# tqch/ddpm-torch

Hardware: AMD Instinct MI355X
Metric: training imgs/s/GPU + 1000-step DDPM samples/s, CIFAR-10 UNet @1/2/4/8 MI355X (higher is better)
Workload: dtype bf16

## Files before the change

### ddpm-torch_amd/csrc/conv3x3.hip

```cpp
#include "common.h"
#include <string.h>
#include <stdlib.h>

namespace {

typedef float f32x4v __attribute__((ext_vector_type(4)));
typedef unsigned u32x2 __attribute__((ext_vector_type(2)));

struct CsArgs {
    const bf16_t* x; long long x_ld; unsigned x_extent;
    const bf16_t* w; unsigned w_extent;
    bf16_t* out; long long out_ld;
    const float* bias; const float* rowbias; long long rowbias_ld; unsigned rowbias_extent;
    const bf16_t* res; long long res_ld;
    int accumulate;
    int B, H, W, C, N, K;
    int ups;
    int tiles_y, tiles_x, tiles_n, total_tiles, xcd;
    FastDiv d_tiles_n, d_tpi, d_tiles_x;
};

template <int PATCH> struct Geo;
template <> struct Geo<16> {
    static constexpr int HWD = 18, HP = 324, LP = 4;
    static constexpr int NI = 6;
    static constexpr int RING = 4;
    static constexpr int WM = 4, NIB = 2, NJ = 2;
    static constexpr int HALO_BYTES = 5 * 512 * 16 + 1024;
};
template <> struct Geo<8> {
    static constexpr int HWD = 10, HP = 100, LP = 3;
    static constexpr int NI = 2;
    static constexpr int RING = 6;
    static constexpr int WM = 2, NIB = 1, NJ = 1;
    static constexpr int HALO_BYTES = 2 * 512 * 16;
};
constexpr int WT_BYTES = 128 * 128;
template <int PATCH> struct Lds {
    static constexpr int DUMP_AT = 2 * Geo<PATCH>::HALO_BYTES + Geo<PATCH>::RING * WT_BYTES;
    static constexpr int ROWS_AT = DUMP_AT + 1024;
    static constexpr int BYTES = ROWS_AT + 4096;
    static_assert(BYTES <= 160 * 1024, "LDS");
};

struct TilePos { int img, py0, px0, tn; };

#ifdef C3_TRACE
__device__ unsigned long long* g_c3_trace = nullptr;
#define C3_TR(id) asm volatile("s_memtime %0" : "=s"(tr_now[id]))
#ifndef C3_TRACE_FIRST
#define C3_TRACE_FIRST 5
#endif
#else
#define C3_TR(id)
#endif
#ifdef C3_TIMING
__device__ unsigned long long* g_c3_timing = nullptr;
#define C3_STAMP(slot) do { if (g_c3_timing && threadIdx.x == 0) g_c3_timing[blockIdx.x * 8 + (slot)] = (slot) == 0 || (slot) == 7 ? wall_clock64() : clock64(); } while (0)
#else
#define C3_STAMP(slot)
#endif

template <int PATCH>
__global__ __launch_bounds__(512, 2)
void conv3x3_stream_kernel(CsArgs a) {
    typedef Geo<PATCH> G_;
    constexpr int HWD = G_::HWD, HP = G_::HP, LP = G_::LP, NI = G_::NI, RING = G_::RING, WM = G_::WM, NIB = G_::NIB, NJ = G_::NJ;
    constexpr int HALO_BYTES = G_::HALO_BYTES, DUMP_AT = Lds<PATCH>::DUMP_AT, ROWS_AT = Lds<PATCH>::ROWS_AT;
    C3_STAMP(0); C3_STAMP(1);
    extern __shared__ __attribute__((aligned(16))) char smem[];
    char* halo = smem;
    char* wring = smem + 2 * HALO_BYTES;
    const int tid = threadIdx.x, lane = tid & 63;
    const int wave = __builtin_amdgcn_readfirstlane(tid >> 6);
    const int wn = wave / WM, wm = wave % WM;

    const __amdgpu_buffer_rsrc_t rx = buffer_rsrc(a.x, a.x_extent), rw = buffer_rsrc(a.w, a.w_extent);
    const __amdgpu_buffer_rsrc_t rbias = buffer_rsrc(a.bias ? (const void*)a.bias : (const void*)a.w, a.bias ? (unsigned)(a.N * 4) : 0u);
    const __amdgpu_buffer_rsrc_t rrow = buffer_rsrc(a.rowbias ? (const void*)a.rowbias : (const void*)a.w, a.rowbias ? a.rowbias_extent : 0u);

    const bool extra = a.res || a.accumulate;
    const int G = gridDim.x;
    const int my_tiles = a.total_tiles > (int)blockIdx.x ? (a.total_tiles - 1 - (int)blockIdx.x) / G + 1 : 0;
    if (my_tiles == 0) return;
    auto tile_pos = [&](int k) {
        const int lid = xcd_logical_id(blockIdx.x + k * G, a.total_tiles, a.xcd);
        const int tmi = (int)fdiv((unsigned)lid, a.d_tiles_n);
        const int tpi = a.tiles_y * a.tiles_x;
        const int img = (int)fdiv((unsigned)tmi, a.d_tpi), pt = tmi - img * tpi;
        const int ty = (int)fdiv((unsigned)pt, a.d_tiles_x);
        TilePos t; t.img = img; t.py0 = ty * PATCH; t.px0 = (pt - ty * a.tiles_x) * PATCH; t.tn = lid - tmi * a.tiles_n;
        return t;
    };
    auto halo_plan = [&](const TilePos& t, unsigned (&ho)[NI]) {
        int tid_ = tid;
        asm volatile("" : "+v"(tid_));
#pragma unroll
        for (int i = 0; i < NI; ++i) {
            const int v = tid_ + 512 * i, hp = v >> 3;
            const int hy = hp / HWD, hx = hp - hy * HWD;
            const int iy = t.py0 + hy - 1, ix = t.px0 + hx - 1;
            const bool ok = hp < HP && (unsigned)iy < (unsigned)a.H && (unsigned)ix < (unsigned)a.W;
            const int lc = (v & 7) ^ (PATCH == 16 ? (hx >> 1) & 7 : ((hx >> 1) ^ ((hy & 1) << 2)) & 7);
            const int sy = iy >> a.ups, sx = ix >> a.ups;
            ho[i] = ok ? ((unsigned)((t.img * (a.H >> a.ups) + sy) * (a.W >> a.ups) + sx) * (unsigned)a.x_ld + (unsigned)(lc * 8)) * 2u : BUF_OOB;
        }
    };
    auto halo_part_off = [&](const TilePos& t, int i) {
        int tid_ = tid;
        asm volatile("" : "+v"(tid_));
        const int v = tid_ + 512 * i, hp = v >> 3;
        const int hy = hp / HWD, hx = hp - hy * HWD;
        const int iy = t.py0 + hy - 1, ix = t.px0 + hx - 1;
        const bool ok = hp < HP && (unsigned)iy < (unsigned)a.H && (unsigned)ix < (unsigned)a.W;
        const int lc = (v & 7) ^ (PATCH == 16 ? (hx >> 1) & 7 : ((hx >> 1) ^ ((hy & 1) << 2)) & 7);
        const int sy = iy >> a.ups, sx = ix >> a.ups;
        return ok ? ((unsigned)((t.img * (a.H >> a.ups) + sy) * (a.W >> a.ups) + sx) * (unsigned)a.x_ld + (unsigned)(lc * 8)) * 2u : BUF_OOB;
    };
    auto issue_halo_part = [&](unsigned ho, int i, int cc, char* dst) {
        const unsigned o = ho == BUF_OOB ? BUF_OOB : ho + (unsigned)(cc * 128);
        char* d = (PATCH == 8 || i < 5) ? dst + (wave * 64 + 512 * i) * 16 : (wave == 0 ? dst + 5 * 512 * 16 : smem + DUMP_AT);
        LDS_DMA16(rx, d, o, 0);
    };
    unsigned wrow[2];
#pragma unroll
    for (int i = 0; i < 2; ++i) {
        const int v = tid + 512 * i, row = v >> 3, lc = (v & 7) ^ ((row >> 1) & 7);
        wrow[i] = (unsigned)(((long long)row * a.K + lc * 8) * 2);
    }
    const unsigned w_tile_bytes = (unsigned)((long long)128 * a.K * 2);
    const int nchunks = a.C >> 6;
    const int steps_per_tile = nchunks * 9, total = my_tiles * steps_per_tile;

    auto issue_w = [&](int tn, int cc, int tap, int slot) {
        char* dst = wring + slot * WT_BYTES;
        const unsigned base = (unsigned)tn * w_tile_bytes + (unsigned)((tap * a.C + cc * 64) * 2);
#pragma unroll
        for (int i = 0; i < 2; ++i)
            LDS_DMA16(rw, dst + (wave * 64 + 512 * i) * 16, base + wrow[i], 0);
    };
    auto issue_w_half = [&](int tn, int cc, int tap, int slot, int i) {
        char* dst = wring + slot * WT_BYTES;
        const unsigned base = (unsigned)tn * w_tile_bytes + (unsigned)((tap * a.C + cc * 64) * 2);
        LDS_DMA16(rw, dst + (wave * 64 + 512 * i) * 16, base + wrow[i], 0);
    };
    auto issue_rows = [&](const TilePos& t, int parity) {
        char* slot = smem + ROWS_AT + parity * 2048;
        if (wave == 0 && a.bias)
            LDS_DMA16(rbias, slot, lane < 32 ? (unsigned)((t.tn * 128 + lane * 4) * 4) : BUF_OOB, 0);
        if (wave == 1 && a.rowbias)
            LDS_DMA16(rrow, slot + 1024, lane < 32 ? (unsigned)(((long long)t.img * a.rowbias_ld + t.tn * 128 + lane * 4) * 4) : BUF_OOB, 0);
    };

    int hp0[NJ], pxl[NJ], pyl[NJ];
#pragma unroll
    for (int j = 0; j < NJ; ++j) {
        const int p = wm * (32 * NJ) + j * 32 + (lane & 31);
        hp0[j] = (p >> LP) * HWD + (p & (PATCH - 1));
        pxl[j] = p & (PATCH - 1); pyl[j] = (p >> LP) & 1;
    }
    f32x16 acc[NIB][NJ];
#pragma unroll
    for (int i = 0; i < NIB; ++i)
#pragma unroll
        for (int j = 0; j < NJ; ++j) acc[i][j] = (f32x16)(0.f);

    TilePos cur = tile_pos(0);
    unsigned hoff[NI];
    halo_plan(cur, hoff);
#pragma unroll
    for (int i = 0; i < NI; ++i) issue_halo_part(hoff[i], i, 0, halo);
    issue_rows(cur, 0);
#pragma unroll
    for (int t = 0; t < RING - 1; ++t) issue_w(cur.tn, 0, t, t);
    wait_vm<2 * (RING - 2)>();
    __builtin_amdgcn_s_barrier();

    C3_STAMP(2);
    const int sw = (lane >> 5) ^ ((lane >> 1) & 7);
    const int hi = lane >> 5;
    const unsigned lds0 = lds_addr(smem);
    unsigned wv[NIB], hv[NJ];
#pragma unroll
    for (int i = 0; i < NIB; ++i) wv[i] = lds0 + 2 * HALO_BYTES + (unsigned)((wn * (32 * NIB) + i * 32 + (lane & 31)) * 128 + (sw << 4));
#pragma unroll
    for (int j = 0; j < NJ; ++j) hv[j] = lds0 + (unsigned)(hp0[j] * 128);
    u32x4 fw[2][NIB], fx[2][NJ];
    bool pend = false;
#ifdef C3_TRACE
    int trace_step = 0;
    unsigned long long tr_now[16], tr_keep[4][16];
#pragma unroll
    for (int q = 0; q < 4; ++q)
#pragma unroll
        for (int i = 0; i < 16; ++i) tr_keep[q][i] = 0;
#endif
    int slot = 0, hb = 0;
    constexpr int ST = NIB * (32 * NJ / 16);
    bool st8 = false;
    for (int k = 0; k < my_tiles; ++k) {
        const bool more_tiles = k + 1 < my_tiles;
        TilePos nxt = cur;
        if (more_tiles) nxt = tile_pos(k + 1);
        for (int cc = 0; cc < nchunks; ++cc) {
            const char* hcur = halo + hb * HALO_BYTES;
            char* hnxt = halo + (hb ^ 1) * HALO_BYTES;
            const bool same_tile = cc + 1 < nchunks;
            const bool prefetch = same_tile || more_tiles;
            const bool last_chunk = !same_tile;
            const int ncc = same_tile ? cc + 1 : 0;
            const int ntn = same_tile ? cur.tn : nxt.tn;
            u32x2 rv[NJ][NIB][4];
            bool pre = false;
#pragma unroll
            for (int tap = 0; tap < 9; ++tap) {
                const int r = tap / 3, s = tap - 3 * r;
                const int shift = r * HWD + s;
                const unsigned woff = (unsigned)(slot * WT_BYTES);
                const unsigned hoffs = (unsigned)(hb * HALO_BYTES + shift * 128);
                unsigned hk[NJ], wk[NIB];
#pragma unroll
                for (int j = 0; j < NJ; ++j) {
                    int px = pxl[j];
                    asm volatile("" : "+v"(px));
                    const int key = PATCH == 16 ? ((px + s) >> 1) & 7 : (((px + s) >> 1) ^ (((pyl[j] + r) & 1) << 2)) & 7;
                    hk[j] = hv[j] + hoffs + (unsigned)((hi ^ key) << 4);
                }
#pragma unroll
                for (int i = 0; i < NIB; ++i) { wk[i] = wv[i]; asm volatile("" : "+v"(wk[i])); }
                auto sub_step = [&](bool mf, const u32x4 (&cw)[NIB], const u32x4 (&cx)[NJ], int kc, u32x4 (&nw)[NIB], u32x4 (&nx)[NJ]) {
                    auto rd_w = [&](int i) {
                        if (kc < 0) return;
                        const unsigned ad = (wk[i] ^ (unsigned)(kc << 5)) + woff;
                        asm volatile("ds_read_b128 %0, %1" : "=v"(nw[i]) : "v"(ad) : "memory");
                        __builtin_amdgcn_sched_barrier(0);
                    };
                    auto rd_x = [&](int j) {
                        if (kc < 0) return;
                        const unsigned ad = hk[j] ^ (unsigned)(kc << 5);
                        asm volatile("ds_read_b128 %0, %1" : "=v"(nx[j]) : "v"(ad) : "memory");
                        __builtin_amdgcn_sched_barrier(0);
                    };
                    auto mm = [&](int i, int j) {
                        if (!mf) return;
                        acc[i][j] = __builtin_amdgcn_mfma_f32_32x32x16_bf16(__builtin_bit_cast(bf16x8, cw[i]), __builtin_bit_cast(bf16x8, cx[j]), acc[i][j], 0, 0, 0);
                        __builtin_amdgcn_sched_barrier(0);
                    };
                    if constexpr (NIB == 2 && NJ == 2) {
                        rd_w(0); mm(0, 0); rd_x(0); mm(0, 1); rd_x(1); mm(1, 0); rd_w(1); mm(1, 1);
                    } else {
                        static_assert(NIB == 1 && NJ == 1, "interleave pattern");
                        rd_w(0); mm(0, 0); rd_x(0);
                    }
                };
#define C3_WAIT_SET() do { asm volatile("s_waitcnt lgkmcnt(0)" ::: "memory"); __builtin_amdgcn_sched_barrier(0); } while (0)
                C3_TR(0);
                sub_step(tap > 0 || pend, fw[1], fx[1], 0, fw[0], fx[0]);
                C3_TR(1);
                if (tap == 8 && last_chunk && extra) {
                    pre = true;
                    const int n0 = cur.tn * 128 + wn * (32 * NIB) + 4 * (lane >> 5);
#pragma unroll
                    for (int j = 0; j < NJ; ++j) {
                        const int p = wm * (32 * NJ) + j * 32 + (lane & 31);
                        const bf16_t* base = (a.res ? a.res : a.out) + ((long long)(cur.img * a.H + cur.py0 + (p >> LP)) * a.W + cur.px0 + (p & (PATCH - 1))) * (a.res ? a.res_ld : a.out_ld)
                                             + (n0 < a.N ? n0 : 0);
#pragma unroll
                        for (int i = 0; i < NIB; ++i)
#pragma unroll
                            for (int g = 0; g < 4; ++g)
                                asm volatile("global_load_dwordx2 %0, %1, off offset:%2" : "=v"(rv[j][i][g]) : "v"(base), "n"((i * 32 + 8 * g) * 2) : "memory");
                    }
                }
                if (tap == 9 - (RING - 1) && last_chunk && prefetch) issue_rows(nxt, (k + 1) & 1);
                const int wslot = slot + RING - 1 >= RING ? slot - 1 : slot + RING - 1;
                if (tap + RING - 1 < 9) issue_w_half(cur.tn, cc, tap + RING - 1, wslot, 0);
                else if (prefetch) issue_w_half(ntn, ncc, tap + RING - 1 - 9, wslot, 0);
                __builtin_amdgcn_sched_barrier(0);
                C3_TR(2);
                C3_WAIT_SET();
                C3_TR(3);
                sub_step(true, fw[0], fx[0], 1, fw[1], fx[1]);
                C3_TR(4);
                if (tap + RING - 1 < 9) issue_w_half(cur.tn, cc, tap + RING - 1, wslot, 1);
                else if (prefetch) issue_w_half(ntn, ncc, tap + RING - 1 - 9, wslot, 1);
                __builtin_amdgcn_sched_barrier(0);
                C3_TR(5);
                C3_WAIT_SET();
                C3_TR(6);
                sub_step(true, fw[1], fx[1], 2, fw[0], fx[0]);
                C3_TR(7);
                if (tap < NI && prefetch) {
                    if (last_chunk) hoff[tap < NI ? tap : 0] = halo_part_off(nxt, tap);
                    issue_halo_part(hoff[tap < NI ? tap : 0], tap, ncc, hnxt);
                }
                __builtin_amdgcn_sched_barrier(0);
                C3_TR(8);
                C3_WAIT_SET();
                C3_TR(9);
                sub_step(true, fw[0], fx[0], 3, fw[1], fx[1]);
                C3_TR(10);
                if (tap == 8 && last_chunk) {
                    asm volatile("s_waitcnt lgkmcnt(0)" ::: "memory");
                    __builtin_amdgcn_s_barrier();
                    __builtin_amdgcn_sched_barrier(0);
                    sub_step(true, fw[1], fx[1], -1, fw[0], fx[0]);
                    pend = false;
                } else pend = true;
#undef C3_WAIT_SET
                slot = slot + 1 == RING ? 0 : slot + 1;
                if (tap == 8 && last_chunk) break;
                if (!prefetch && 7 - tap < RING - 2) {
                    if (7 - tap >= 3) wait_vm<6>(); else if (7 - tap == 2) wait_vm<4>(); else if (7 - tap == 1) wait_vm<2>(); else wait_vm<0>();
                }
                else {
                    int hp = 0;
                    if (prefetch) {
#pragma unroll
                        for (int b = 0; b <= RING - 2; ++b) hp += (tap - b >= 0 && tap - b < NI) ? 1 : 0;
                    }
                    static_assert(RING - 2 <= 4, "hp cases");
                    if (tap < RING - 2 && cc == 0 && st8) {
                        if (hp >= 3) wait_vm<2 * (RING - 2) + ST + 3>(); else if (hp == 2) wait_vm<2 * (RING - 2) + ST + 2>(); else if (hp == 1) wait_vm<2 * (RING - 2) + ST + 1>(); else wait_vm<2 * (RING - 2) + ST>();
                    } else {
                        if (hp >= 3) wait_vm<2 * (RING - 2) + 3>(); else if (hp == 2) wait_vm<2 * (RING - 2) + 2>(); else if (hp == 1) wait_vm<2 * (RING - 2) + 1>(); else wait_vm<2 * (RING - 2)>();
                    }
                }
                C3_TR(11);
                asm volatile("s_waitcnt lgkmcnt(0)" ::: "memory");
                C3_TR(12);
                __builtin_amdgcn_s_barrier();
                C3_TR(13);
#ifdef C3_TRACE
                asm volatile("s_waitcnt lgkmcnt(0)" ::: "memory");
#pragma unroll
                for (int q = 0; q < 4; ++q)
                    if (trace_step == C3_TRACE_FIRST + q) {
#pragma unroll
                        for (int i = 0; i < 14; ++i) tr_keep[q][i] = tr_now[i];
                    }
                ++trace_step;
#endif
            }
            if (last_chunk) {
                if (k == 0) C3_STAMP(3); else if (k == 1) C3_STAMP(5);
                const char* rows = smem + ROWS_AT + (k & 1) * 2048;
                if (pre) {
                    if (prefetch) wait_vm<2>(); else wait_vm<0>();
                    __builtin_amdgcn_sched_barrier(0);
                    if (!(cur.tn * 128 + wn * (32 * NIB) < a.N)) {
#pragma unroll
                        for (int j = 0; j < NJ; ++j)
#pragma unroll
                            for (int i = 0; i < NIB; ++i)
#pragma unroll
                                for (int g = 0; g < 4; ++g) rv[j][i][g] = (u32x2)(0u);
                    }
                }
                const int n0 = cur.tn * 128 + wn * (32 * NIB);
                constexpr int STG_PX = 32 * NJ, NRR = STG_PX / 16;
                const unsigned stg = lds0 + (unsigned)(hb * HALO_BYTES + wave * (STG_PX * 64));
                static_assert(8 * STG_PX * 64 <= HALO_BYTES, "staging slices fit the halo buffer");
                bf16_t* const obase = a.out + ((long long)(cur.img * a.H + cur.py0) * a.W + cur.px0) * a.out_ld + n0 + 8 * (lane & 3);
                auto orow = [&](int rr) {
                    int q = lane >> 2;
                    asm volatile("" : "+v"(q));
                    const int p = wm * STG_PX + rr * 16 + q;
                    return obase + (long long)(((p >> LP) * a.W + (p & (PATCH - 1))) * (int)a.out_ld);
                };
#pragma unroll
                for (int i = 0; i < NIB; ++i) {
                    f32x4v bsum[4], brow[4];
#pragma unroll
                    for (int g = 0; g < 4; ++g) {
                        const unsigned ad = lds_addr(rows + (wn * (32 * NIB) + i * 32 + 8 * g + 4 * (lane >> 5)) * 4);
                        asm volatile("ds_read_b128 %0, %1" : "=v"(bsum[g]) : "v"(ad) : "memory");
                        asm volatile("ds_read_b128 %0, %1 offset:1024" : "=v"(brow[g]) : "v"(ad) : "memory");
                    }
                    asm volatile("s_waitcnt lgkmcnt(0)" ::: "memory");
                    __builtin_amdgcn_sched_barrier(0);
#pragma unroll
                    for (int g = 0; g < 4; ++g) {
                        if (!a.bias) bsum[g] = (f32x4v)(0.f);
                        if (!a.rowbias) brow[g] = (f32x4v)(0.f);
                    }
#pragma unroll
                    for (int j = 0; j < NJ; ++j) {
                        uint2 pk[4];
#pragma unroll
                        for (int g = 0; g < 4; ++g) {
                            float v[4] = {acc[i][j][4 * g], acc[i][j][4 * g + 1], acc[i][j][4 * g + 2], acc[i][j][4 * g + 3]};
                            v[0] += bsum[g].x + brow[g].x; v[1] += bsum[g].y + brow[g].y;
                            v[2] += bsum[g].z + brow[g].z; v[3] += bsum[g].w + brow[g].w;
                            if (extra) {
                                const u32x2 r2 = rv[j][i][g];
                                v[0] += __uint_as_float(r2.x << 16); v[1] += __uint_as_float(r2.x & 0xffff0000u);
                                v[2] += __uint_as_float(r2.y << 16); v[3] += __uint_as_float(r2.y & 0xffff0000u);
                            }
                            pk[g].x = pack_bf2(v[0], v[1]); pk[g].y = pack_bf2(v[2], v[3]);
                        }
#pragma unroll
                        for (int q2 = 0; q2 < 2; ++q2) {
                            const u32x2 sx = __builtin_amdgcn_permlane32_swap(pk[2 * q2].x, pk[2 * q2 + 1].x, false, false);
                            const u32x2 sy = __builtin_amdgcn_permlane32_swap(pk[2 * q2].y, pk[2 * q2 + 1].y, false, false);
                            u32x4 o; o.x = sx.x; o.y = sy.x; o.z = sx.y; o.w = sy.y;
                            const int P = j * 32 + (lane & 31), sl = (2 * q2 + hi) ^ ((P >> 2) & 3);
                            const unsigned ad = stg + (unsigned)(P * 64 + (sl << 4));
                            asm volatile("ds_write_b128 %0, %1" :: "v"(ad), "v"(o) : "memory");
                        }
                    }
                    u32x4 back[NRR];
#pragma unroll
                    for (int rr = 0; rr < NRR; ++rr) {
                        const int Q = rr * 16 + (lane >> 2), sl = (lane & 3) ^ ((Q >> 2) & 3);
                        const unsigned ad = stg + (unsigned)(Q * 64 + (sl << 4));
                        asm volatile("ds_read_b128 %0, %1" : "=v"(back[rr]) : "v"(ad) : "memory");
                    }
                    asm volatile("s_waitcnt lgkmcnt(0)" ::: "memory");
                    __builtin_amdgcn_sched_barrier(0);
                    if (n0 < a.N) {
#pragma unroll
                        for (int rr = 0; rr < NRR; ++rr) {
#ifdef C3_NO_STORE
                            if (back[rr].x == 0x12345678u)
#endif
                            *reinterpret_cast<u32x4*>(orow(rr) + i * 32) = back[rr];
                        }
                    }
                }
#pragma unroll
                for (int i = 0; i < NIB; ++i)
#pragma unroll
                    for (int j = 0; j < NJ; ++j) acc[i][j] = (f32x16)(0.f);
                if (k == 0) C3_STAMP(4); else if (k == 1) C3_STAMP(6);
                st8 = n0 < a.N;
                if (!more_tiles) wait_vm<0>(); else if (st8) wait_vm<2 * (RING - 2) + ST>(); else wait_vm<2 * (RING - 2)>();
                asm volatile("s_waitcnt lgkmcnt(0)" ::: "memory");
                __builtin_amdgcn_s_barrier();
            }
            hb ^= 1;
        }
        cur = nxt;
    }
    C3_STAMP(7);
#ifdef C3_TRACE
    if (g_c3_trace && blockIdx.x == 0 && (wave & 3) == 0 && lane == 0) {
#pragma unroll
        for (int q = 0; q < 4; ++q)
#pragma unroll
            for (int i = 0; i < 16; ++i) g_c3_trace[((wave >> 2) * 64 + q) * 16 + i] = tr_keep[q][i];
    }
#endif
}


constexpr int PC_CNT_AT = Lds<16>::BYTES;
constexpr int PC_BYTES = PC_CNT_AT + 1024;
static_assert(PC_BYTES <= 160 * 1024, "LDS");
constexpr int PC_READY = 0, PC_FREED = 16, PC_EDONE = 32, PC_JUNK = 256;

__device__ unsigned g_pc_fault[4];

#ifdef C3_TIMING
#define PC_STAMP(slot) do { if (g_c3_timing && threadIdx.x == 0) g_c3_timing[blockIdx.x * 8 + (slot)] = (slot) == 0 || (slot) == 7 ? wall_clock64() : clock64(); } while (0)
#define PC_STEP() do { if (g_c3_timing && threadIdx.x == 0 && tstep < 64) g_c3_timing[2048 + blockIdx.x * 64 + tstep] = clock64(); ++tstep; } while (0)
#else
#define PC_STAMP(slot)
#define PC_STEP()
#endif
__global__ __launch_bounds__(512, 2)
void conv3x3_pc_kernel(CsArgs a) {
    typedef Geo<16> G_;
    constexpr int HWD = G_::HWD, HP = G_::HP, RING = G_::RING;
    constexpr int HALO_BYTES = G_::HALO_BYTES, DUMP_AT = Lds<16>::DUMP_AT, ROWS_AT = Lds<16>::ROWS_AT;
    constexpr int NP = 11;
    static_assert(RING == 4, "the vmcnt tables below are written for a ring of four");
    extern __shared__ __attribute__((aligned(16))) char smem[];
    char* halo = smem;
    char* wring = smem + 2 * HALO_BYTES;
    const int tid = threadIdx.x, lane = tid & 63;
    const int wave = __builtin_amdgcn_readfirstlane(tid >> 6);
    const int G = gridDim.x;
    const int my_tiles = a.total_tiles > (int)blockIdx.x ? (a.total_tiles - 1 - (int)blockIdx.x) / G + 1 : 0;
    if (my_tiles == 0) return;
    if (tid < 256) reinterpret_cast<unsigned*>(smem + PC_CNT_AT)[tid] = 0u;
    __syncthreads();
    auto tile_pos = [&](int k) {
        const int lid = xcd_logical_id(blockIdx.x + k * G, a.total_tiles, a.xcd);
        const int tmi = (int)fdiv((unsigned)lid, a.d_tiles_n);
        const int tpi = a.tiles_y * a.tiles_x;
        const int img = (int)fdiv((unsigned)tmi, a.d_tpi), pt = tmi - img * tpi;
        const int ty = (int)fdiv((unsigned)pt, a.d_tiles_x);
        TilePos t; t.img = img; t.py0 = ty * 16; t.px0 = (pt - ty * a.tiles_x) * 16; t.tn = lid - tmi * a.tiles_n;
        return t;
    };
    const int nchunks = a.C >> 6;
    const unsigned lds0 = lds_addr(smem);
    const unsigned cnt0 = lds0 + PC_CNT_AT, junk = cnt0 + PC_JUNK + (unsigned)(lane * 4);

    if (wave >= 4) {
        const int lw = wave - 4, lid = lw * 64 + lane;
        const __amdgpu_buffer_rsrc_t rx = buffer_rsrc(a.x, a.x_extent), rw = buffer_rsrc(a.w, a.w_extent);
        const __amdgpu_buffer_rsrc_t rbias = buffer_rsrc(a.bias ? (const void*)a.bias : (const void*)a.w, a.bias ? (unsigned)(a.N * 4) : 0u);
        const __amdgpu_buffer_rsrc_t rrow = buffer_rsrc(a.rowbias ? (const void*)a.rowbias : (const void*)a.w, a.rowbias ? a.rowbias_extent : 0u);
        auto halo_part_off = [&](const TilePos& t, int p) {
            int lid_ = lid;
            asm volatile("" : "+v"(lid_));
            const int v = lid_ + 256 * p, hp = v >> 3;
            const int hy = hp / HWD, hx = hp - hy * HWD;
            const int iy = t.py0 + hy - 1, ix = t.px0 + hx - 1;
            const bool ok = hp < HP && (unsigned)iy < (unsigned)a.H && (unsigned)ix < (unsigned)a.W;
            const int lc = (v & 7) ^ ((hx >> 1) & 7);
            const int sy = iy >> a.ups, sx = ix >> a.ups;
            return ok ? ((unsigned)((t.img * (a.H >> a.ups) + sy) * (a.W >> a.ups) + sx) * (unsigned)a.x_ld + (unsigned)(lc * 8)) * 2u : BUF_OOB;
        };
        auto issue_halo_part = [&](const TilePos& t, int p, int cc, char* dst) {
            const unsigned ho = halo_part_off(t, p);
            const unsigned o = ho == BUF_OOB ? BUF_OOB : ho + (unsigned)(cc * 128);
            char* d = p < 10 ? dst + (lw * 64 + 256 * p) * 16 : (lw == 0 ? dst + 2560 * 16 : smem + DUMP_AT);
            LDS_DMA16(rx, d, o, 0);
        };
        unsigned wrow[4];
#pragma unroll
        for (int i = 0; i < 4; ++i) {
            const int v = lid + 256 * i, row = v >> 3, lc = (v & 7) ^ ((row >> 1) & 7);
            wrow[i] = (unsigned)(((long long)row * a.K + lc * 8) * 2);
        }
        const unsigned w_tile_bytes = (unsigned)((long long)128 * a.K * 2);
        auto issue_w = [&](int tn, int cc, int tap, int slot) {
            char* dst = wring + slot * WT_BYTES;
            const unsigned base = (unsigned)tn * w_tile_bytes + (unsigned)((tap * a.C + cc * 64) * 2);
#pragma unroll
            for (int i = 0; i < 4; ++i)
                LDS_DMA16(rw, dst + (lw * 64 + 256 * i) * 16, base + wrow[i], 0);
        };
        auto issue_rows = [&](const TilePos& t, int parity) {
            char* slot = smem + ROWS_AT + parity * 2048;
            if (lw == 0)
                LDS_DMA16(rbias, slot, (lane < 32 && a.bias) ? (unsigned)((t.tn * 128 + lane * 4) * 4) : BUF_OOB, 0);
            else if (lw == 1)
                LDS_DMA16(rrow, slot + 1024, (lane < 32 && a.rowbias) ? (unsigned)(((long long)t.img * a.rowbias_ld + t.tn * 128 + lane * 4) * 4) : BUF_OOB, 0);
            else
                LDS_DMA16(rw, smem + DUMP_AT, BUF_OOB, 0);
        };
        TilePos cur = tile_pos(0);
#pragma unroll
        for (int p = 0; p < NP; ++p) issue_halo_part(cur, p, 0, halo);
        issue_rows(cur, 0);
#pragma unroll
        for (int t = 0; t < RING - 1; ++t) issue_w(cur.tn, 0, t, t);
        const unsigned sig_ready = lane == 0 ? cnt0 + PC_READY + (unsigned)(lw * 4) : junk;
        wait_vm<8>();
        lds_signal(sig_ready);
        int slot = 0, hb = 0;
        unsigned gstep = 0;
        for (int k = 0; k < my_tiles; ++k) {
            const bool more_tiles = k + 1 < my_tiles;
            TilePos nxt = cur;
            if (more_tiles) nxt = tile_pos(k + 1);
            for (int cc = 0; cc < nchunks; ++cc) {
                char* hnxt = halo + (hb ^ 1) * HALO_BYTES;
                const bool same_tile = cc + 1 < nchunks;
                const bool prefetch = same_tile || more_tiles;
                const bool last_chunk = !same_tile;
                const int ncc = same_tile ? cc + 1 : 0;
                const int ntn = same_tile ? cur.tn : nxt.tn;
                const bool rows_here = last_chunk && prefetch;
#pragma unroll
                for (int tap = 0; tap < 9; ++tap) {
                    lds_wait_all_ge(g_pc_fault, cnt0 + PC_FREED, gstep);
                    if (prefetch && tap < 6) {
                        if (tap < 5) { issue_halo_part(same_tile ? cur : nxt, 2 * tap, ncc, hnxt); issue_halo_part(same_tile ? cur : nxt, 2 * tap + 1, ncc, hnxt); }
                        else issue_halo_part(same_tile ? cur : nxt, 10, ncc, hnxt);
                    }
                    if (tap == 6 && rows_here) issue_rows(nxt, (k + 1) & 1);
                    const int wslot = slot + RING - 1 >= RING ? slot - 1 : slot + RING - 1;
                    if (tap + RING - 1 < 9) issue_w(cur.tn, cc, tap + RING - 1, wslot);
                    else if (prefetch) issue_w(ntn, ncc, tap + RING - 1 - 9, wslot);
                    slot = slot + 1 == RING ? 0 : slot + 1;
                    if (prefetch) {
                        if (tap == 0) wait_vm<10>();
                        else if (tap < 5) wait_vm<12>();
                        else if (tap == 5) wait_vm<11>();
                        else if (tap == 6) { if (rows_here) wait_vm<10>(); else wait_vm<9>(); }
                        else if (tap == 7) { if (rows_here) wait_vm<9>(); else wait_vm<8>(); }
                        else wait_vm<8>();
                    } else {
                        if (tap < 6) wait_vm<8>(); else if (tap == 6) wait_vm<4>(); else wait_vm<0>();
                    }
                    lds_signal(sig_ready);
                    ++gstep;
                }
                hb ^= 1;
            }
            cur = nxt;
        }
        return;
    }

    constexpr int NIB = 2, NJ = 4;
    const int wn = wave >> 1, wm = wave & 1;
    f32x16 acc[NIB][NJ];
    const int sw = (lane >> 5) ^ ((lane >> 1) & 7);
    const int hi = lane >> 5;
    constexpr int XJ = 2 * HWD * 128, WI = 32 * 128;
    const unsigned wv0 = lds0 + 2 * HALO_BYTES + (unsigned)((wn * 64 + (lane & 31)) * 128 + (sw << 4));
    unsigned kx[3];
    {
        const int p = wm * 128 + (lane & 31), px = p & 15;
        const unsigned hv0 = lds0 + (unsigned)(((p >> 4) * HWD + px) * 128);
#pragma unroll
        for (int s_ = 0; s_ < 3; ++s_) kx[s_] = hv0 + (unsigned)(s_ * 128) + (unsigned)((hi ^ (((px + s_) >> 1) & 7)) << 4);
    }
    auto init_acc = [&](int parity) {
        const char* rows = smem + ROWS_AT + parity * 2048;
#pragma unroll
        for (int i = 0; i < NIB; ++i) {
            f32x4v bsum[4], brow[4];
#pragma unroll
            for (int g = 0; g < 4; ++g) {
                const unsigned ad = lds_addr(rows + (wn * 64 + i * 32 + 8 * g + 4 * (lane >> 5)) * 4);
                asm volatile("ds_read_b128 %0, %1" : "=v"(bsum[g]) : "v"(ad) : "memory");
                asm volatile("ds_read_b128 %0, %1 offset:1024" : "=v"(brow[g]) : "v"(ad) : "memory");
            }
            asm volatile("s_waitcnt lgkmcnt(0)" ::: "memory");
            __builtin_amdgcn_sched_barrier(0);
#pragma unroll
            for (int g = 0; g < 4; ++g) {
                const f32x4v sum = bsum[g] + brow[g];
#pragma unroll
                for (int j = 0; j < NJ; ++j) { acc[i][j][4 * g] = sum.x; acc[i][j][4 * g + 1] = sum.y; acc[i][j][4 * g + 2] = sum.z; acc[i][j][4 * g + 3] = sum.w; }
            }
        }
    };
    auto halo_addr = [&](int tap_, int hb_) {
        const int r = tap_ / 3, s_ = tap_ - 3 * r;
        unsigned v = kx[s_] + (unsigned)(hb_ * HALO_BYTES + r * HWD * 128);
        asm volatile("" : "+v"(v));
        return v;
    };
    auto w_addr = [&](int slot_) { unsigned v = wv0 + (unsigned)(slot_ * WT_BYTES); asm volatile("" : "+v"(v)); return v; };
    u32x4 fw[2][NIB], fx[2][NJ];
    unsigned hk, wk, hkn = 0, wkn = 0;
    u32x4 rcp = {0u, 0u, 0u, 0u};
    const unsigned sig_freed = lane == 0 ? cnt0 + PC_FREED + (unsigned)(wave * 4) : junk;
    const unsigned sig_edone = lane == 0 ? cnt0 + PC_EDONE : junk;
    TilePos cur = tile_pos(0);
#ifdef C3_TIMING
    int tstep = 0;
#endif
    PC_STAMP(0); PC_STAMP(1);
    unsigned need = 1;
    lds_wait_all_ge(g_pc_fault, cnt0 + PC_READY, need);
    PC_STAMP(2);
    init_acc(0);
    int slot = 0, hb = 0;
    hk = halo_addr(0, 0);
    wk = w_addr(0);
    bool pend = false;
    for (int k = 0; k < my_tiles; ++k) {
        for (int cc = 0; cc < nchunks; ++cc) {
            const bool last_chunk = cc + 1 == nchunks;
#pragma unroll
            for (int tap = 0; tap < 9; ++tap) {
                const bool tile_end = tap == 8 && last_chunk;
                const int nslot = slot + 1 == RING ? 0 : slot + 1;
                auto sub_step = [&](bool mf, const u32x4 (&cw)[NIB], const u32x4 (&cx)[NJ], int kc, u32x4 (&nw)[NIB], u32x4 (&nx)[NJ], int pre, int post, unsigned sig, bool nextaddr) {
                    unsigned aw = 0, ax = 0;
                    if (kc >= 0) { aw = wk ^ (unsigned)(kc << 5); ax = hk ^ (unsigned)(kc << 5); }
                    const int rd = kc >= 0 ? 1 : 0;
                    auto rd_w = [&](int i) {
                        if (kc < 0) return;
                        asm volatile("ds_read_b128 %0, %1 offset:%2" : "=v"(nw[i]) : "v"(aw), "n"(i * WI) : "memory");
                        __builtin_amdgcn_sched_barrier(0);
                    };
                    auto rd_x = [&](int j) {
                        if (kc < 0) return;
                        asm volatile("ds_read_b128 %0, %1 offset:%2" : "=v"(nx[j]) : "v"(ax), "n"(j * XJ) : "memory");
                        __builtin_amdgcn_sched_barrier(0);
                    };
                    auto mm = [&](int i, int j) {
                        if (!mf) return;
                        acc[i][j] = __builtin_amdgcn_mfma_f32_32x32x16_bf16(__builtin_bit_cast(bf16x8, cw[i]), __builtin_bit_cast(bf16x8, cx[j]), acc[i][j], 0, 0, 0);
                        __builtin_amdgcn_sched_barrier(0);
                    };
                    auto wl = [&](int n) {
                        if (!mf) return;
                        switch (n) {
                            case 0: asm volatile("s_waitcnt lgkmcnt(0)" ::: "memory"); break;
                            case 1: asm volatile("s_waitcnt lgkmcnt(1)" ::: "memory"); break;
                            case 2: asm volatile("s_waitcnt lgkmcnt(2)" ::: "memory"); break;
                            case 3: asm volatile("s_waitcnt lgkmcnt(3)" ::: "memory"); break;
                            case 4: asm volatile("s_waitcnt lgkmcnt(4)" ::: "memory"); break;
                            case 5: asm volatile("s_waitcnt lgkmcnt(5)" ::: "memory"); break;
                            case 6: asm volatile("s_waitcnt lgkmcnt(6)" ::: "memory"); break;
                            case 7: asm volatile("s_waitcnt lgkmcnt(7)" ::: "memory"); break;
                            case 8: asm volatile("s_waitcnt lgkmcnt(8)" ::: "memory"); break;
                            default: asm volatile("s_waitcnt lgkmcnt(9)" ::: "memory"); break;
                        }
                        __builtin_amdgcn_sched_barrier(0);
                    };
                    const int po = post ? 1 : 0;
                    wl(4 + pre);
                    mm(0, 0); rd_w(0); rd_x(0);
                    wl(3 + pre + 2 * rd);
                    mm(1, 0); rd_w(1); rd_x(1);
                    wl(2 + pre + 4 * rd);
                    mm(0, 1); rd_x(2); rd_x(3);
                    if (post == 1) {
                        asm volatile("ds_read_b128 %0, %1" : "=v"(rcp) : "v"(cnt0 + PC_READY) : "memory");
                        __builtin_amdgcn_sched_barrier(0);
                    } else if (post == 2) {
                        lds_signal(sig);
                        __builtin_amdgcn_sched_barrier(0);
                    }
                    mm(1, 1);
                    if (nextaddr) {
                        hkn = tap < 8 ? halo_addr(tap + 1, hb) : halo_addr(0, hb ^ 1);
                        wkn = w_addr(nslot);
                        __builtin_amdgcn_sched_barrier(0);
                    }
                    wl(1 + pre + 6 * rd + po);
                    mm(0, 2); mm(1, 2);
                    wl(pre + 6 * rd + po);
                    mm(0, 3); mm(1, 3);
                };
                if (tap > 0 || pend) {
                    asm volatile("s_waitcnt lgkmcnt(5)" ::: "memory");
                    __builtin_amdgcn_sched_barrier(0);
                    if (lds_min_dist(rcp, need) < 0) lds_wait_all_ge(g_pc_fault, cnt0 + PC_READY, need);
                }
                sub_step(tap > 0 || pend, fw[1], fx[1], 0, fw[0], fx[0], 1, 0, 0u, false);
                sub_step(true, fw[0], fx[0], 1, fw[1], fx[1], 0, 0, 0u, false);
                sub_step(true, fw[1], fx[1], 2, fw[0], fx[0], 0, 1, 0u, false);
                sub_step(true, fw[0], fx[0], 3, fw[1], fx[1], 1, 2, tile_end ? sig_edone : sig_freed, !tile_end);
                slot = nslot;
                need += 1;
                if (tile_end) {
                    sub_step(true, fw[1], fx[1], -1, fw[0], fx[0], 1, 0, 0u, false);
                    pend = false;
                    if (k == 0) PC_STAMP(3); else if (k == 1) PC_STAMP(5);
                    lds_wait_ge(g_pc_fault, cnt0 + PC_EDONE, 4u * (unsigned)(k + 1));
                    break;
                }
                pend = true;
                hk = hkn; wk = wkn;
                if (tap == 8) { asm volatile("s_waitcnt lgkmcnt(0)" ::: "memory"); __builtin_amdgcn_sched_barrier(0); }
                PC_STEP();
            }
            if (last_chunk) {
                const int n0 = cur.tn * 128 + wn * 64;
                const bool live = n0 < a.N;
                const unsigned stg = lds0 + (unsigned)(hb * HALO_BYTES + wave * (64 * 64));
                const unsigned long long ob =
                    (unsigned long long)(a.out + ((long long)(cur.img * a.H + cur.py0 + wm * 8) * a.W + cur.px0) * a.out_ld + n0);
                const unsigned ob_lo = __builtin_amdgcn_readfirstlane((unsigned)ob), ob_hi = __builtin_amdgcn_readfirstlane((unsigned)(ob >> 32));
                const unsigned long long obase = ((unsigned long long)ob_hi << 32) | ob_lo;
                const unsigned rowstride = (unsigned)__builtin_amdgcn_readfirstlane((int)(a.W * (int)a.out_ld * 2));
                const unsigned loff = (unsigned)(((lane >> 2) * (int)a.out_ld + 8 * (lane & 3)) * 2);
                typedef __attribute__((address_space(1))) u32x4 gvec_t;
                auto orow = [&](int q16, int col) { return (gvec_t*)(obase + (unsigned long long)q16 * rowstride + (unsigned)(col * 2)) + 0; };
#pragma unroll
                for (int i = 0; i < NIB; ++i) {
#pragma unroll
                    for (int jh = 0; jh < 2; ++jh) {
#pragma unroll
                        for (int jj = 0; jj < 2; ++jj) {
                            const int j = 2 * jh + jj;
                            uint2 pk[4];
#pragma unroll
                            for (int g = 0; g < 4; ++g) {
                                float v[4] = {acc[i][j][4 * g], acc[i][j][4 * g + 1], acc[i][j][4 * g + 2], acc[i][j][4 * g + 3]};
                                pk[g].x = pack_bf2(v[0], v[1]); pk[g].y = pack_bf2(v[2], v[3]);
                            }
#pragma unroll
                            for (int q2 = 0; q2 < 2; ++q2) {
                                const u32x2 sx = __builtin_amdgcn_permlane32_swap(pk[2 * q2].x, pk[2 * q2 + 1].x, false, false);
                                const u32x2 sy = __builtin_amdgcn_permlane32_swap(pk[2 * q2].y, pk[2 * q2 + 1].y, false, false);
                                u32x4 o; o.x = sx.x; o.y = sy.x; o.z = sx.y; o.w = sy.y;
                                const int P = jj * 32 + (lane & 31), sl = (2 * q2 + hi) ^ ((P >> 2) & 3);
                                const unsigned ad = stg + (unsigned)(P * 64 + (sl << 4));
                                asm volatile("ds_write_b128 %0, %1" :: "v"(ad), "v"(o) : "memory");
                            }
                        }
                        u32x4 back[4];
#pragma unroll
                        for (int rr = 0; rr < 4; ++rr) {
                            const int Q = rr * 16 + (lane >> 2), sl = (lane & 3) ^ ((Q >> 2) & 3);
                            const unsigned ad = stg + (unsigned)(Q * 64 + (sl << 4));
                            asm volatile("ds_read_b128 %0, %1" : "=v"(back[rr]) : "v"(ad) : "memory");
                        }
                        asm volatile("s_waitcnt lgkmcnt(0)" ::: "memory");
                        __builtin_amdgcn_sched_barrier(0);
                        if (live) {
#pragma unroll
                            for (int rr = 0; rr < 4; ++rr) *(gvec_t*)((__attribute__((address_space(1))) char*)orow(jh * 4 + rr, i * 32) + loff) = back[rr];
                        }
                    }
                }
                lds_signal(sig_freed);
                if (k + 1 < my_tiles) {
                    cur = tile_pos(k + 1);
                    lds_wait_all_ge(g_pc_fault, cnt0 + PC_READY, need);
                    init_acc((k + 1) & 1);
                    hk = halo_addr(0, hb ^ 1);
                    wk = w_addr(slot);
                }
                PC_STEP();
                if (k == 0) PC_STAMP(4); else if (k == 1) PC_STAMP(6);
            }
            hb ^= 1;
        }
    }
    PC_STAMP(7);
}


}

#ifdef C3_TRACE
extern "C" int ddpm_debug_set_c3_trace(void* p) { return hipMemcpyToSymbol(HIP_SYMBOL(g_c3_trace), &p, sizeof(p)) == hipSuccess ? 0 : -1; }
#endif
#ifdef C3_TIMING
extern "C" int ddpm_debug_set_c3_timing(void* p) { return hipMemcpyToSymbol(HIP_SYMBOL(g_c3_timing), &p, sizeof(p)) == hipSuccess ? 0 : -1; }
#endif

extern "C" int ddpm_conv3x3_pc_last_fault(unsigned* out4) {
    if (!out4) return DDPM_ERR_NULL;
    return hipMemcpyFromSymbol(out4, HIP_SYMBOL(g_pc_fault), 4 * sizeof(unsigned)) == hipSuccess ? DDPM_OK : DDPM_ERR_LAUNCH;
}

int ddpm_conv3x3_stream_launch(const void* x, long long x_ld, const void* w, void* y, long long y_ld, const float* bias, const float* rowbias,
                               long long rowbias_ld, const void* residual, long long res_ld, int accumulate, int B, int H, int W, int C, int N,
                               int upsample, int xcd, int dry, void* stream) {
    const long long M = (long long)B * H * W;
    const int patch = (H % 16 == 0 && W % 16 == 0 && M >= 16384) ? 16 : ((H % 8 == 0 && W % 8 == 0 && M >= 4096) ? 8 : 0);
    if (!patch || (residual && accumulate) || C % 64 || N % 64 || x_ld % 8 || y_ld % 8 || (residual && res_ld % 4) || (rowbias && rowbias_ld % 4)) return -1;
    if (!aligned16(x) || !aligned16(w) || !aligned16(y) || (residual && (((uintptr_t)residual) & 7)) || (bias && !aligned16(bias)) || (rowbias && !aligned16(rowbias))) return -1;
    if (upsample && ((H | W) & 1)) return -1;
    const long long xbytes = ((long long)B * (H >> upsample) * (W >> upsample) * x_ld - (x_ld - C)) * 2, wbytes = (long long)N * 9 * C * 2;
    const long long rbbytes = rowbias ? ((long long)(B - 1) * rowbias_ld + N) * 4 : 0;
    if (xbytes > BUF_OOB || wbytes > BUF_OOB || rbbytes > BUF_OOB) return -1;
    const bool use_pc = patch == 16 && !residual && !accumulate;
    if (dry) return use_pc ? 17 : patch;
    CsArgs a; memset(&a, 0, sizeof(a));
    a.x = (const bf16_t*)x; a.x_ld = x_ld; a.x_extent = (unsigned)xbytes;
    a.w = (const bf16_t*)w; a.w_extent = (unsigned)wbytes;
    a.out = (bf16_t*)y; a.out_ld = y_ld;
    a.bias = bias; a.rowbias = rowbias; a.rowbias_ld = rowbias_ld; a.rowbias_extent = (unsigned)rbbytes;
    a.res = (const bf16_t*)residual; a.res_ld = res_ld; a.accumulate = accumulate;
    a.B = B; a.H = H; a.W = W; a.C = C; a.N = N; a.K = 9 * C; a.ups = upsample ? 1 : 0;
    a.tiles_y = H / patch; a.tiles_x = W / patch; a.tiles_n = (N + 127) / 128;
    a.total_tiles = B * a.tiles_y * a.tiles_x * a.tiles_n;
    a.xcd = xcd;
    a.d_tiles_n = make_fastdiv((unsigned)a.tiles_n); a.d_tpi = make_fastdiv((unsigned)(a.tiles_y * a.tiles_x)); a.d_tiles_x = make_fastdiv((unsigned)a.tiles_x);
    const int cus = ddpm_cu_budget(256);
    const int grid = a.total_tiles < cus ? a.total_tiles : cus;
#define C3_LAUNCH(PATCHV)                                                                                                              \
    do {                                                                                                                               \
        static DevOnce attr_set;                                                                                                  \
        if (!attr_set) {                                                                                                               \
            if (hipFuncSetAttribute(reinterpret_cast<const void*>(&conv3x3_stream_kernel<PATCHV>), hipFuncAttributeMaxDynamicSharedMemorySize, \
                                    Lds<PATCHV>::BYTES) != hipSuccess) return DDPM_ERR_LAUNCH;                                         \
            attr_set = true;                                                                                                           \
        }                                                                                                                              \
        hipLaunchKernelGGL(conv3x3_stream_kernel<PATCHV>, dim3(grid), dim3(512), Lds<PATCHV>::BYTES, (hipStream_t)stream, a);           \
    } while (0)
    if (use_pc) {
        static DevOnce pc_attr_set;
        if (!pc_attr_set) {
            if (hipFuncSetAttribute(reinterpret_cast<const void*>(&conv3x3_pc_kernel), hipFuncAttributeMaxDynamicSharedMemorySize, PC_BYTES) != hipSuccess) return DDPM_ERR_LAUNCH;
            pc_attr_set = true;
        }
        hipLaunchKernelGGL(conv3x3_pc_kernel, dim3(grid), dim3(512), PC_BYTES, (hipStream_t)stream, a);
    }
    else if (patch == 16) C3_LAUNCH(16); else C3_LAUNCH(8);
#undef C3_LAUNCH
    return check_launch();
}
```

### ddpm-torch_amd/csrc/probe.hip

```cpp
#include "common.h"

namespace {

__global__ __launch_bounds__(256) void mfma_probe_kernel(float* sink, int iters, unsigned seed, int zero) {
    const unsigned id = blockIdx.x * 256 + threadIdx.x;
    u32x4 a[4], b[4];
#pragma unroll
    for (int i = 0; i < 8; ++i) {
        unsigned w[4];
#pragma unroll
        for (int c = 0; c < 4; ++c) {
            const unsigned h = mix32(seed ^ mix32(id * 32u + i * 4u + c));
            const unsigned lo = ((h & 1u) << 15) | ((124u + ((h >> 1) % 6u)) << 7) | ((h >> 4) & 127u);
            const unsigned hi = (((h >> 11) & 1u) << 15) | ((124u + ((h >> 12) % 6u)) << 7) | ((h >> 16) & 127u);
            w[c] = zero ? 0u : (lo | (hi << 16));
        }
        const u32x4 v = {w[0], w[1], w[2], w[3]};
        if (i < 4) a[i] = v; else b[i - 4] = v;
    }
    f32x16 acc[8];
#pragma unroll
    for (int i = 0; i < 8; ++i) acc[i] = (f32x16)(0.f);
#define MM(m, ai, bi) acc[m] = __builtin_amdgcn_mfma_f32_32x32x16_bf16(__builtin_bit_cast(bf16x8, a[ai]), __builtin_bit_cast(bf16x8, b[bi]), acc[m], 0, 0, 0)
    for (int it = 0; it < iters; ++it) {
        MM(0, 0, 0); MM(1, 1, 0); MM(2, 0, 1); MM(3, 1, 1); MM(4, 0, 2); MM(5, 1, 2); MM(6, 0, 3); MM(7, 1, 3);
        MM(0, 2, 0); MM(1, 3, 0); MM(2, 2, 1); MM(3, 3, 1); MM(4, 2, 2); MM(5, 3, 2); MM(6, 2, 3); MM(7, 3, 3);
    }
#undef MM
    float s = 0.f;
#pragma unroll
    for (int i = 0; i < 8; ++i)
#pragma unroll
        for (int r = 0; r < 16; ++r) s += acc[i][r];
    if (s == 12345.678f) sink[threadIdx.x] = s;
}

__global__ __launch_bounds__(512) void copy_probe_kernel(u32x4* dst, const u32x4* src, long long vecs) {
    for (long long i = (long long)blockIdx.x * 512 + threadIdx.x; i < vecs; i += (long long)gridDim.x * 512)
        __builtin_nontemporal_store(__builtin_nontemporal_load(src + i), dst + i);
}

}

static std::atomic<int> g_reserved_cus{0};
int ddpm_reserved_cus() { return g_reserved_cus.load(std::memory_order_relaxed); }
extern "C" int ddpm_set_reserved_cus(int n) {
    if (n < 0 || n > 192) return DDPM_ERR_SHAPE;
    g_reserved_cus.store(n, std::memory_order_relaxed);
    return DDPM_OK;
}
extern "C" int ddpm_get_reserved_cus(void) { return ddpm_reserved_cus(); }

extern "C" int ddpm_copy_probe(void* dst, const void* src, long long bytes, int blocks, void* stream) {
    if (!dst || !src) return DDPM_ERR_NULL;
    if (bytes <= 0 || bytes % 16 || blocks <= 0 || blocks > 4096) return DDPM_ERR_SHAPE;
    if (!aligned16(dst) || !aligned16(src)) return DDPM_ERR_ALIGN;
    hipLaunchKernelGGL(copy_probe_kernel, dim3(blocks), dim3(512), 0, (hipStream_t)stream, (u32x4*)dst, (const u32x4*)src, bytes / 16);
    return check_launch();
}

extern "C" int ddpm_mfma_probe(float* sink, int iters, int zero_operands, void* stream) {
    if (!sink) return DDPM_ERR_NULL;
    if (iters <= 0) return DDPM_ERR_SHAPE;
    hipLaunchKernelGGL(mfma_probe_kernel, dim3(256), dim3(256), 0, (hipStream_t)stream, sink, iters, 0x9E3779B9u, zero_operands);
    return check_launch();
}
```

Measured before the change: 14530.

## Offload conv3x3 epilogue global stores to producer waves via LDS staging handshake

In the producer/consumer conv3x3 kernel, the compute waves used to read their staged output back from LDS and issue the global stores themselves. Now they only write packed results into double-buffered staging slices and signal a new STAGED counter. The loader waves read those slices and issue the global stores at the start of the next tile, signalling DRAINED so the compute waves can reuse the slices. This moves store latency off the MFMA waves at the cost of extra LDS counter handshakes, adjusted vmcnt/lgkmcnt tables and tighter coupling between the wave groups. It also adds timing stamps and relaxes the reserved-CU bound.

```diff
diff --git a/ddpm-torch_amd/csrc/conv3x3.hip b/ddpm-torch_amd/csrc/conv3x3.hip
--- a/ddpm-torch_amd/csrc/conv3x3.hip
+++ b/ddpm-torch_amd/csrc/conv3x3.hip
@@ -457,16 +457,22 @@
 constexpr int PC_CNT_AT = Lds<16>::BYTES;
 constexpr int PC_BYTES = PC_CNT_AT + 1024;
 static_assert(PC_BYTES <= 160 * 1024, "LDS");
-constexpr int PC_READY = 0, PC_FREED = 16, PC_EDONE = 32, PC_JUNK = 256;
+constexpr int PC_READY = 0, PC_FREED = 16, PC_EDONE = 32, PC_STAGED = 48, PC_DRAINED = 64, PC_JUNK = 256;
+constexpr int PC_STAGE_BYTES = 2 * 64 * 64;
+static_assert(4 * PC_STAGE_BYTES <= Geo<16>::HALO_BYTES, "the staging slices live in the finished halo buffer");
 
 __device__ unsigned g_pc_fault[4];
 
 #ifdef C3_TIMING
 #define PC_STAMP(slot) do { if (g_c3_timing && threadIdx.x == 0) g_c3_timing[blockIdx.x * 8 + (slot)] = (slot) == 0 || (slot) == 7 ? wall_clock64() : clock64(); } while (0)
 #define PC_STEP() do { if (g_c3_timing && threadIdx.x == 0 && tstep < 64) g_c3_timing[2048 + blockIdx.x * 64 + tstep] = clock64(); ++tstep; } while (0)
+#define PC_LSTAMP(t, s) do { if (g_c3_timing && threadIdx.x == 256 && (t) < 2) g_c3_timing[2048 + 256 * 64 + blockIdx.x * 8 + 4 * (t) + (s)] = clock64(); } while (0)
+#define PC_BSTAMP(t, s) do { if (g_c3_timing && threadIdx.x == 0 && (t) < 2) g_c3_timing[2048 + 256 * 64 + 2048 + blockIdx.x * 8 + 4 * (t) + (s)] = clock64(); } while (0)
 #else
 #define PC_STAMP(slot)
 #define PC_STEP()
+#define PC_LSTAMP(t, s)
+#define PC_BSTAMP(t, s)
 #endif
 __global__ __launch_bounds__(512, 2)
 void conv3x3_pc_kernel(CsArgs a) {
@@ -543,7 +549,48 @@
             else
                 LDS_DMA16(rw, smem + DUMP_AT, BUF_OOB, 0);
         };
-        TilePos cur = tile_pos(0);
+        const unsigned sig_drained = lane == 0 ? cnt0 + PC_DRAINED + (unsigned)(lw * 4) : junk;
+        unsigned npiece = 0;
+        auto serve = [&](const TilePos& t, int hbuf, int tk) {
+            const int cwn = lw >> 1, cwm = lw & 1;
+            const int n0 = t.tn * 128 + cwn * 64;
+            const bool live = n0 < a.N;
+            const unsigned long long ob =
+                (unsigned long long)(a.out + ((long long)(t.img * a.H + t.py0 + cwm * 8) * a.W + t.px0) * a.out_ld + n0);
+            const unsigned ob_lo = __builtin_amdgcn_readfirstlane((unsigned)ob), ob_hi = __builtin_amdgcn_readfirstlane((unsigned)(ob >> 32));
+            const unsigned long long obase = ((unsigned long long)ob_hi << 32) | ob_lo;
+            const unsigned rowstride = (unsigned)__builtin_amdgcn_readfirstlane((int)(a.W * (int)a.out_ld * 2));
+            const unsigned loff = (unsigned)(((lane >> 2) * (int)a.out_ld + 8 * (lane & 3)) * 2);
+            const unsigned stg = lds0 + (unsigned)(hbuf * HALO_BYTES + lw * PC_STAGE_BYTES);
+#pragma unroll
+            for (int p = 0; p < 4; ++p) {
+                const int i = p >> 1, jh = p & 1;
+                lds_wait_ge(g_pc_fault, cnt0 + PC_STAGED + (unsigned)(lw * 4), npiece + (unsigned)p + 1u);
+                if (p == 0) PC_LSTAMP(tk, 0);
+                u32x4 back[4];
+#pragma unroll
+                for (int rr = 0; rr < 4; ++rr) {
+                    const int Q = rr * 16 + (lane >> 2), sl = (lane & 3) ^ ((Q >> 2) & 3);
+                    const unsigned ad = stg + (unsigned)((p & 1) * 4096 + Q * 64 + (sl << 4));
+                    asm volatile("ds_read_b128 %0, %1" : "=v"(back[rr]) : "v"(ad) : "memory");
+                }
+                asm volatile("s_waitcnt lgkmcnt(0)" ::: "memory");
+                __builtin_amdgcn_sched_barrier(0);
+                lds_signal(sig_drained);
+                if (p == 3) PC_LSTAMP(tk, 1);
+                if (live) {
+#pragma unroll
+                    for (int rr = 0; rr < 4; ++rr) {
+                        const unsigned long long rb = obase + (unsigned long long)(jh * 4 + rr) * rowstride + (unsigned)(i * 64);
+                        asm volatile("global_store_dwordx4 %0, %1, %2" :: "v"(loff), "v"(back[rr]), "s"(rb) : "memory");
+                    }
+                }
+            }
+            npiece += 4;
+            PC_LSTAMP(tk, 2);
+            return live;
+        };
+        TilePos cur = tile_pos(0), prv = cur;
 #pragma unroll
         for (int p = 0; p < NP; ++p) issue_halo_part(cur, p, 0, halo);
         issue_rows(cur, 0);
@@ -566,9 +613,15 @@
                 const int ncc = same_tile ? cc + 1 : 0;
                 const int ntn = same_tile ? cur.tn : nxt.tn;
                 const bool rows_here = last_chunk && prefetch;
+                bool st16 = false;
 #pragma unroll
                 for (int tap = 0; tap < 9; ++tap) {
                     lds_wait_all_ge(g_pc_fault, cnt0 + PC_FREED, gstep);
+                    if (tap == 0 && cc == 0 && k > 0) {
+                        st16 = serve(prv, hb ^ 1, k - 1);
+                        lds_wait_all_ge(g_pc_fault, cnt0 + PC_DRAINED, npiece);
+                        PC_LSTAMP(k - 1, 3);
+                    }
                     if (prefetch && tap < 6) {
                         if (tap < 5) { issue_halo_part(same_tile ? cur : nxt, 2 * tap, ncc, hnxt); issue_halo_part(same_tile ? cur : nxt, 2 * tap + 1, ncc, hnxt); }
                         else issue_halo_part(same_tile ? cur : nxt, 10, ncc, hnxt);
@@ -578,7 +631,10 @@
                     if (tap + RING - 1 < 9) issue_w(cur.tn, cc, tap + RING - 1, wslot);
                     else if (prefetch) issue_w(ntn, ncc, tap + RING - 1 - 9, wslot);
                     slot = slot + 1 == RING ? 0 : slot + 1;
-                    if (prefetch) {
+                    if (st16 && tap < 2) {
+                        if (prefetch) { if (tap == 0) wait_vm<10 + 16>(); else wait_vm<12 + 16>(); }
+                        else wait_vm<8 + 16>();
+                    } else if (prefetch) {
                         if (tap == 0) wait_vm<10>();
                         else if (tap < 5) wait_vm<12>();
                         else if (tap == 5) wait_vm<11>();
@@ -593,8 +649,10 @@
                 }
                 hb ^= 1;
             }
+            prv = cur;
             cur = nxt;
         }
+        serve(prv, hb ^ 1, my_tiles - 1);
         return;
     }
 
@@ -645,7 +703,7 @@
     u32x4 rcp = {0u, 0u, 0u, 0u};
     const unsigned sig_freed = lane == 0 ? cnt0 + PC_FREED + (unsigned)(wave * 4) : junk;
     const unsigned sig_edone = lane == 0 ? cnt0 + PC_EDONE : junk;
-    TilePos cur = tile_pos(0);
+    const unsigned sig_staged = lane == 0 ? cnt0 + PC_STAGED + (unsigned)(wave * 4) : junk;
 #ifdef C3_TIMING
     int tstep = 0;
 #endif
@@ -665,7 +723,7 @@
             for (int tap = 0; tap < 9; ++tap) {
                 const bool tile_end = tap == 8 && last_chunk;
                 const int nslot = slot + 1 == RING ? 0 : slot + 1;
-                auto sub_step = [&](bool mf, const u32x4 (&cw)[NIB], const u32x4 (&cx)[NJ], int kc, u32x4 (&nw)[NIB], u32x4 (&nx)[NJ], int pre, int post, unsigned sig, bool nextaddr) {
+                auto sub_step = [&](bool mf, const u32x4 (&cw)[NIB], const u32x4 (&cx)[NJ], int kc, u32x4 (&nw)[NIB], u32x4 (&nx)[NJ], int pre, int post, unsigned sig, bool nextaddr, bool two = false, unsigned sig2 = 0u) {
                     unsigned aw = 0, ax = 0;
                     if (kc >= 0) { aw = wk ^ (unsigned)(kc << 5); ax = hk ^ (unsigned)(kc << 5); }
                     const int rd = kc >= 0 ? 1 : 0;
@@ -696,11 +754,12 @@
                             case 6: asm volatile("s_waitcnt lgkmcnt(6)" ::: "memory"); break;
                             case 7: asm volatile("s_waitcnt lgkmcnt(7)" ::: "memory"); break;
                             case 8: asm volatile("s_waitcnt lgkmcnt(8)" ::: "memory"); break;
-                            default: asm volatile("s_waitcnt lgkmcnt(9)" ::: "memory"); break;
+                            case 9: asm volatile("s_waitcnt lgkmcnt(9)" ::: "memory"); break;
+                            default: asm volatile("s_waitcnt lgkmcnt(10)" ::: "memory"); break;
                         }
                         __builtin_amdgcn_sched_barrier(0);
                     };
-                    const int po = post ? 1 : 0;
+                    const int po = post ? (two ? 2 : 1) : 0;
                     wl(4 + pre);
                     mm(0, 0); rd_w(0); rd_x(0);
                     wl(3 + pre + 2 * rd);
@@ -712,6 +771,7 @@
                         __builtin_amdgcn_sched_barrier(0);
                     } else if (post == 2) {
                         lds_signal(sig);
+                        if (two) lds_signal(sig2);
                         __builtin_amdgcn_sched_barrier(0);
                     }
                     mm(1, 1);
@@ -725,19 +785,21 @@
                     wl(pre + 6 * rd + po);
                     mm(0, 3); mm(1, 3);
                 };
+                const int sigs = tap == 0 ? 2 : 1;
                 if (tap > 0 || pend) {
-                    asm volatile("s_waitcnt lgkmcnt(5)" ::: "memory");
+                    if (tap == 0) asm volatile("s_waitcnt lgkmcnt(6)" ::: "memory"); else asm volatile("s_waitcnt lgkmcnt(5)" ::: "memory");
                     __builtin_amdgcn_sched_barrier(0);
                     if (lds_min_dist(rcp, need) < 0) lds_wait_all_ge(g_pc_fault, cnt0 + PC_READY, need);
                 }
-                sub_step(tap > 0 || pend, fw[1], fx[1], 0, fw[0], fx[0], 1, 0, 0u, false);
+                sub_step(tap > 0 || pend, fw[1], fx[1], 0, fw[0], fx[0], sigs, 0, 0u, false);
                 sub_step(true, fw[0], fx[0], 1, fw[1], fx[1], 0, 0, 0u, false);
                 sub_step(true, fw[1], fx[1], 2, fw[0], fx[0], 0, 1, 0u, false);
-                sub_step(true, fw[0], fx[0], 3, fw[1], fx[1], 1, 2, tile_end ? sig_edone : sig_freed, !tile_end);
+                if (tap == 8) sub_step(true, fw[0], fx[0], 3, fw[1], fx[1], 1, 2, tile_end ? sig_edone : junk, !tile_end, true, sig_freed);
+                else sub_step(true, fw[0], fx[0], 3, fw[1], fx[1], 1, 2, sig_freed, true);
                 slot = nslot;
                 need += 1;
                 if (tile_end) {
-                    sub_step(true, fw[1], fx[1], -1, fw[0], fx[0], 1, 0, 0u, false);
+                    sub_step(true, fw[1], fx[1], -1, fw[0], fx[0], 2, 0, 0u, false);
                     pend = false;
                     if (k == 0) PC_STAMP(3); else if (k == 1) PC_STAMP(5);
                     lds_wait_ge(g_pc_fault, cnt0 + PC_EDONE, 4u * (unsigned)(k + 1));
@@ -749,21 +811,14 @@
                 PC_STEP();
             }
             if (last_chunk) {
-                const int n0 = cur.tn * 128 + wn * 64;
-                const bool live = n0 < a.N;
-                const unsigned stg = lds0 + (unsigned)(hb * HALO_BYTES + wave * (64 * 64));
-                const unsigned long long ob =
-                    (unsigned long long)(a.out + ((long long)(cur.img * a.H + cur.py0 + wm * 8) * a.W + cur.px0) * a.out_ld + n0);
-                const unsigned ob_lo = __builtin_amdgcn_readfirstlane((unsigned)ob), ob_hi = __builtin_amdgcn_readfirstlane((unsigned)(ob >> 32));
-                const unsigned long long obase = ((unsigned long long)ob_hi << 32) | ob_lo;
-                const unsigned rowstride = (unsigned)__builtin_amdgcn_readfirstlane((int)(a.W * (int)a.out_ld * 2));
-                const unsigned loff = (unsigned)(((lane >> 2) * (int)a.out_ld + 8 * (lane & 3)) * 2);
-                typedef __attribute__((address_space(1))) u32x4 gvec_t;
-                auto orow = [&](int q16, int col) { return (gvec_t*)(obase + (unsigned long long)q16 * rowstride + (unsigned)(col * 2)) + 0; };
+                PC_BSTAMP(k, 0);
+                const unsigned stg = lds0 + (unsigned)(hb * HALO_BYTES + wave * PC_STAGE_BYTES);
 #pragma unroll
                 for (int i = 0; i < NIB; ++i) {
 #pragma unroll
                     for (int jh = 0; jh < 2; ++jh) {
+                        const int p = 2 * i + jh;
+                        u32x4 o[2][2];
 #pragma unroll
                         for (int jj = 0; jj < 2; ++jj) {
                             const int j = 2 * jh + jj;
@@ -777,31 +832,25 @@
                             for (int q2 = 0; q2 < 2; ++q2) {
                                 const u32x2 sx = __builtin_amdgcn_permlane32_swap(pk[2 * q2].x, pk[2 * q2 + 1].x, false, false);
                                 const u32x2 sy = __builtin_amdgcn_permlane32_swap(pk[2 * q2].y, pk[2 * q2 + 1].y, false, false);
-                                u32x4 o; o.x = sx.x; o.y = sy.x; o.z = sx.y; o.w = sy.y;
-                                const int P = jj * 32 + (lane & 31), sl = (2 * q2 + hi) ^ ((P >> 2) & 3);
-                                const unsigned ad = stg + (unsigned)(P * 64 + (sl << 4));
-                                asm volatile("ds_write_b128 %0, %1" :: "v"(ad), "v"(o) : "memory");
+                                o[jj][q2].x = sx.x; o[jj][q2].y = sy.x; o[jj][q2].z = sx.y; o[jj][q2].w = sy.y;
                             }
                         }
-                        u32x4 back[4];
-#pragma unroll
-                        for (int rr = 0; rr < 4; ++rr) {
-                            const int Q = rr * 16 + (lane >> 2), sl = (lane & 3) ^ ((Q >> 2) & 3);
-                            const unsigned ad = stg + (unsigned)(Q * 64 + (sl << 4));
-                            asm volatile("ds_read_b128 %0, %1" : "=v"(back[rr]) : "v"(ad) : "memory");
-                        }
-                        asm volatile("s_waitcnt lgkmcnt(0)" ::: "memory");
-                        __builtin_amdgcn_sched_barrier(0);
-                        if (live) {
-#pragma unroll
-                            for (int rr = 0; rr < 4; ++rr) *(gvec_t*)((__attribute__((address_space(1))) char*)orow(jh * 4 + rr, i * 32) + loff) = back[rr];
-                        }
-                    }
-                }
-                lds_signal(sig_freed);
+                        if (k > 0 || p >= 2) lds_wait_ge(g_pc_fault, cnt0 + PC_DRAINED + (unsigned)(wave * 4), 4u * (unsigned)k + (unsigned)p - 1u);
+#pragma unroll
+                        for (int jj = 0; jj < 2; ++jj)
+#pragma unroll
+                            for (int q2 = 0; q2 < 2; ++q2) {
+                                const int P = jj * 32 + (lane & 31), sl = (2 * q2 + hi) ^ ((P >> 2) & 3);
+                                const unsigned ad = stg + (unsigned)((p & 1) * 4096 + P * 64 + (sl << 4));
+                                asm volatile("ds_write_b128 %0, %1" :: "v"(ad), "v"(o[jj][q2]) : "memory");
+                            }
+                        lds_signal(sig_staged);
+                    }
+                }
+                PC_BSTAMP(k, 1);
                 if (k + 1 < my_tiles) {
-                    cur = tile_pos(k + 1);
                     lds_wait_all_ge(g_pc_fault, cnt0 + PC_READY, need);
+                    PC_BSTAMP(k, 2);
                     init_acc((k + 1) & 1);
                     hk = halo_addr(0, hb ^ 1);
                     wk = w_addr(slot);
diff --git a/ddpm-torch_amd/csrc/probe.hip b/ddpm-torch_amd/csrc/probe.hip
--- a/ddpm-torch_amd/csrc/probe.hip
+++ b/ddpm-torch_amd/csrc/probe.hip
@@ -45,7 +45,7 @@
 static std::atomic<int> g_reserved_cus{0};
 int ddpm_reserved_cus() { return g_reserved_cus.load(std::memory_order_relaxed); }
 extern "C" int ddpm_set_reserved_cus(int n) {
-    if (n < 0 || n > 192) return DDPM_ERR_SHAPE;
+    if (n < 0 || n > 255) return DDPM_ERR_SHAPE;
     g_reserved_cus.store(n, std::memory_order_relaxed);
     return DDPM_OK;
 }
```

Result: no change. 14500 (-0.2%).
